# XuyangBai/PointDSC

Hardware: AMD Instinct MI355X
Metric: point-cloud pairs/sec @ N=5000 corr (higher is better)
Workload: dtype f32 (attention products as fp16x3 split (fp16 hi+lo operand pairs, three f16 MFMAs per product), f32 accumulate; fc_message / PointCN products as fp16 hi+lo split; spatial-consistency matrix stored as unorm16); 1 GPU; 3DMatch-like synthetic correspondences (BASELINE.json configs[2]): N=5000 corr, 32 pairs per step sharded over 1 GPU(s) = 32 per GPU, 12-layer PointDSC, seeded random weights; num_corr=5000, pairs_per_gpu=32, global_batch=32, compat_format=u16, layer_gemm=h3, att_leaves=canonical, latency_mode=False, range_guard=lazy (pipeline), collective=none (single process, no process group)

## Files before the change

### include/pointdsc_hip.h

```cpp
#ifndef POINTDSC_HIP_H
#define POINTDSC_HIP_H

#include <stddef.h>

#ifdef __cplusplus
extern "C" {
#endif

#define PDSC_VERSION 9
#define PDSC_CHANNELS 128
#define PDSC_MAX_K 64
#define PDSC_MAX_POWER_ITERS 32

enum pdsc_status {
    PDSC_OK = 0,
    PDSC_ERR_ARG = -1,
    PDSC_ERR_WORKSPACE = -2,
    PDSC_ERR_LAUNCH = -3
};

typedef struct pdsc_config {
    int in_dim;
    int num_layers;
    int num_channels;
// ... 84 lines not shown
    PDSC_LAYER_KERNEL_AUTO = 0,
    PDSC_LAYER_KERNEL_BLOCK,
    PDSC_LAYER_KERNEL_WAVE,
    PDSC_LAYER_KERNEL_H3,
    PDSC_LAYER_KERNEL_X3
};
typedef struct pdsc_layer_call {
    const float* msg;
    const float* part_o;
    const float* part_ml;
    int nsplit, Npad;
    const float* res;
    const float* feat_in;
    float* feat_out;
    float* featB_out;
    float* qkv_out;
    void* q_split;
    void* kv_tiles;
    const void* w1; const float* b1;
    const void* w2; const float* b2;
    const void* w3; const float* b3;
    const void* wp; const float* bp;
    const void* wq; const float* bq;
    const void* wq_split;
    const void* wfrag_tail;
    const void* wfrag_head;
    int gemm_format;
    int io_flags;
    int bs, N;
    int kernel;
} pdsc_layer_call;
int pdsc_layer_run(const pdsc_layer_call* call, void* stream);

size_t    pdsc_wsplit_bytes(const pdsc_config* cfg);
long long pdsc_wsplit_offset(const pdsc_config* cfg, int section, int layer);
int       pdsc_wsplit_build(const pdsc_config* cfg, const float* wpack, void* wsplit, void* stream);
#define PDSC_WS_FRAG_TAIL 100
#define PDSC_WS_FRAG_HEAD 101
#define PDSC_WS_FRAG_TAIL_H3 102
#define PDSC_WS_FRAG_HEAD_H3 103
#define PDSC_WS_FOLD_TAIL_H3 104
#define PDSC_WS_FOLD_HEAD_H3 105
#define PDSC_WS_FOLD_W 106
size_t pdsc_wfrag_fold_tail_bytes(void);
size_t pdsc_wfrag_fold_head_bytes(void);
int pdsc_layer_prefers_block(int bs, int N);
int pdsc_layer_h3_uses_coop(int bs, int N);
size_t pdsc_wfrag_tail_bytes(void);
size_t pdsc_wfrag_head_bytes(void);
int pdsc_wfrag_build_tail(const float* w1, const float* b1, const float* w2, const float* b2, const float* w3,
                          const float* b3, void* out, int gemm_format, void* stream);
int pdsc_wfrag_build_head(const float* wp, const float* bp, const float* wq, const float* bq, void* out,
                          int gemm_format, void* stream);

size_t pdsc_attention_scratch_bytes(int bs, int N, int nsplit);
int    pdsc_attention_default_split(int bs, int N);
int    pdsc_sc_attention(const float* qkv, const float* compat, long long ld, float* msg,
                         void* scratch, size_t scratch_bytes, int bs, int N, int nsplit, void* stream);

size_t pdsc_split_q_bytes(int bs, int N);
size_t pdsc_split_kv_bytes(int bs, int N);
int    pdsc_pack_qkv_split(const float* qkv, void* q_split, void* kv_tiles, int bs, int N, void* stream);
size_t pdsc_attention_split_scratch_bytes(int bs, int N, int nsplit);
int    pdsc_attention_split_default_split(int bs, int N);
int    pdsc_attention_leaf_count(int N);
int    pdsc_attention_leaf_plan(int bs, int N, int leaves_mode, int* nsplit, int* nleaf);
// ... 247 lines not shown
```

### pointdsc_amd/_lib.py

```python
from __future__ import annotations

import ctypes as C
import os
from pathlib import Path

PKG = Path(__file__).resolve().parent
LIB_PATH = Path(os.environ.get("POINTDSC_HIP_LIB", PKG / "libpointdsc_hip.so"))


class PointDSCLibraryError(RuntimeError):
    pass


class PdscConfig(C.Structure):
    _fields_ = [
        ("in_dim", C.c_int), ("num_layers", C.c_int), ("num_channels", C.c_int),
        ("num_iterations", C.c_int), ("k", C.c_int), ("refine_iters", C.c_int),
        ("inlier_threshold", C.c_float), ("nms_radius", C.c_float), ("refine_threshold", C.c_float),
        ("attention_precision", C.c_int), ("compat_format", C.c_int), ("layer_gemm", C.c_int),
        ("att_leaves", C.c_int), ("value_fold", C.c_int),
    ]


W_SECTIONS = [
    "LAYER0_W", "LAYER0_B", "PCN_W", "PCN_B", "QKV_W", "QKV_B", "FC1_W", "FC1_B", "FC2_W", "FC2_B",
    "FC3_W", "FC3_B", "CLS1_W", "CLS1_B", "CLS2_W", "CLS2_B", "CLS3_W", "CLS3_B", "SIGMA", "SIGMA_SPAT",
]
W = {name: i for i, name in enumerate(W_SECTIONS)}

_vp, _i, _f, _ll, _sz = C.c_void_p, C.c_int, C.c_float, C.c_longlong, C.c_size_t
_cfgp = C.POINTER(PdscConfig)


class PdscLayerCall(C.Structure):
    _fields_ = (
        [(n, _vp) for n in ("msg", "part_o", "part_ml")] + [("nsplit", _i), ("Npad", _i)] +
        [(n, _vp) for n in ("res", "feat_in", "feat_out", "featB_out", "qkv_out", "q_split", "kv_tiles",
                            "w1", "b1", "w2", "b2", "w3", "b3", "wp", "bp", "wq", "bq", "wq_split", "wfrag_tail", "wfrag_head")] +
        [(n, _i) for n in ("gemm_format", "io_flags", "bs", "N", "kernel")])

SIGNATURES = {
    "pdsc_version": (_i, []),
    "pdsc_set_range_report": (_i, [_vp]),
    "pdsc_last_error": (C.c_char_p, []),
    "pdsc_experiments_enabled": (_i, []),
    "pdsc_wpack_floats": (_ll, [_cfgp]),
    "pdsc_wpack_offset": (_ll, [_cfgp, _i, _i]),
    "pdsc_compat_ld": (_ll, [_i]),
    "pdsc_workspace_bytes": (_sz, [_cfgp, _i, _i, _i]),
    "pdsc_workspace_offset": (_ll, [_cfgp, _i, _i, _i, C.c_char_p]),
    "pdsc_spatial_compat": (_i, [_vp, _vp, _vp, _vp, _vp, _ll, _i, _i, _vp]),
    "pdsc_spatial_compat_u16": (_i, [_vp, _vp, _vp, _vp, _ll, _i, _i, _vp]),
    "pdsc_selftest_exact_math": (_i, [_vp, _f, _vp, _vp, _ll, _vp]),
    "pdsc_selftest_mfma_valu_neighbour": (_i, [_vp, _i, _i, _vp]),
    "pdsc_classifier_hidden": (_i, [_vp, _vp, _vp, _vp, _vp, _vp, _i, _vp]),
    "pdsc_linear": (_i, [_vp, _ll, _vp, _vp, _vp, _ll, _vp, _ll, _i, _i, _i, _i, _vp]),
    "pdsc_layer0": (_i, [_vp, _i, _vp, _vp, _vp, _i, _vp]),
    "pdsc_layer_run": (_i, [C.POINTER(PdscLayerCall), _vp]),
    "pdsc_wsplit_bytes": (_sz, [_cfgp]),
    "pdsc_wsplit_offset": (_ll, [_cfgp, _i, _i]),
    "pdsc_wsplit_build": (_i, [_cfgp, _vp, _vp, _vp]),
    "pdsc_layer_prefers_block": (_i, [_i, _i]),
    "pdsc_layer_h3_uses_coop": (_i, [_i, _i]),
    "pdsc_wfrag_tail_bytes": (_sz, []),
    "pdsc_wfrag_head_bytes": (_sz, []),
    "pdsc_wfrag_fold_tail_bytes": (_sz, []),
    "pdsc_wfrag_fold_head_bytes": (_sz, []),
    "pdsc_wfrag_build_tail": (_i, [_vp] * 7 + [_i, _vp]),
    "pdsc_wfrag_build_head": (_i, [_vp] * 5 + [_i, _vp]),
    "pdsc_sc_attention_split_partials": (_i, [_vp, _vp, _vp, _i, _ll, _vp, _sz, _i, _i, _i, _i, _vp]),
    "pdsc_split_q_bytes": (_sz, [_i, _i]),
    "pdsc_split_kv_bytes": (_sz, [_i, _i]),
    "pdsc_pack_qkv_split": (_i, [_vp, _vp, _vp, _i, _i, _vp]),
    "pdsc_attention_split_scratch_bytes": (_sz, [_i, _i, _i]),
    "pdsc_attention_split_default_split": (_i, [_i, _i]),
    "pdsc_attention_leaf_count": (_i, [_i]),
    "pdsc_attention_leaf_plan": (_i, [_i, _i, _i, C.POINTER(C.c_int), C.POINTER(C.c_int)]),
    "pdsc_attention_leaf_scratch_bytes": (_sz, [_i, _i, _i]),
    "pdsc_attention_trace": (_i, [_vp]),
    "pdsc_attention_leaf_split_override": (_i, [_i]),
    "pdsc_layer_trace": (_i, [_vp]),
    "pdsc_sc_attention_split": (_i, [_vp, _vp, _vp, _ll, _vp, _vp, _sz, _i, _i, _i, _vp]),
    "pdsc_sc_attention_split_u16": (_i, [_vp, _vp, _vp, _ll, _vp, _vp, _sz, _i, _i, _i, _vp]),
    "pdsc_attention_scratch_bytes": (_sz, [_i, _i, _i]),
    "pdsc_attention_default_split": (_i, [_i, _i]),
    "pdsc_sc_attention": (_i, [_vp, _vp, _ll, _vp, _vp, _sz, _i, _i, _i, _vp]),
    "pdsc_normalize_confidence": (_i, [_vp, _vp, _vp, _vp, _vp, _vp, _i, _vp]),
    "pdsc_nms_keys": (_i, [_vp, _vp, _f, _vp, _i, _i, _vp]),
    "pdsc_nms_workspace_bytes": (_sz, [_i, _i]),
    "pdsc_nms_keys_grid": (_i, [_vp, _vp, _f, _vp, _vp, _sz, _i, _i, _vp]),
    "pdsc_rank_select": (_i, [_vp, _vp, _i, _i, _i, _vp]),
# ... 115 lines not shown
```

### pointdsc_amd/csrc/layer.hip

```cpp
#include <stdlib.h>
#include <type_traits>
#include "pdsc_common.h"
#include "split_layout.h"
#include "merge_partials.h"
#include "layer_args.h"
#include "layer_block.h"

namespace pdsc {

constexpr int LF_ROWS = 32;
constexpr int LF_LD = PDSC_CHANNELS + 4;
constexpr int LF_TILE = LF_ROWS * LF_LD;


#define LF_STAMP(k)                                                                                   \
    if (a.trace && lane == 0) a.trace[(((size_t)blockIdx.y * gridDim.x + blockIdx.x) * 4 + wave) * 16 + (k)] = __builtin_readcyclecounter();

template <int K>
__device__ __forceinline__ void load_w(const float* __restrict__ W, int n0, int l31, int h, f32x4 (&w)[K / 8]) {
    const float* p = W + (size_t)(n0 + l31) * K + 4 * h;
#pragma unroll
    for (int q = 0; q < K / 8; ++q) w[q] = *reinterpret_cast<const f32x4*>(p + 8 * q);
}

// ... 321 lines not shown
        profile_mark_end(PDSC_PROF_LAYER, st);
        return rc;
    }
    if (tail) return launch_layer<true, false>(a, st);
    return launch_layer<false, true>(a, st);
}

}

static bool choose_layer_kernel(const pdsc_layer_call& c, const pdsc::LayerArgs& a, pdsc::LayerKernel* kernel) {
    using pdsc::LayerKernel;
    switch (c.kernel) {
        case PDSC_LAYER_KERNEL_BLOCK: *kernel = LayerKernel::Block; return true;
        case PDSC_LAYER_KERNEL_WAVE: *kernel = LayerKernel::Wave; return true;
        case PDSC_LAYER_KERNEL_H3: *kernel = LayerKernel::H3; return true;
        case PDSC_LAYER_KERNEL_X3: *kernel = LayerKernel::X3; return true;
        case PDSC_LAYER_KERNEL_AUTO: break;
        default: return false;
    }
    if (!a.wf_tail && !a.wf_head) {
        const char* ev = pdsc::env_str("PDSC_LAYER_VARIANT");
        const bool block = ev && (ev[0] == 'b' || ev[0] == 'w') ? ev[0] == 'b' : pdsc_layer_prefers_block(c.bs, c.N) != 0;
        *kernel = block ? LayerKernel::Block : LayerKernel::Wave;
    } else if (c.io_flags != 0) {
        *kernel = LayerKernel::H3;
    } else {
        const bool h3 = c.gemm_format == PDSC_LAYER_GEMM_H3 && pdsc::env_int("PDSC_LAYER_H3_VARIANT", 1) != 0 &&
                        pdsc::launch_layer_h3_fits(a, a.msg != nullptr || a.part_o != nullptr, a.featB_out != nullptr);
        *kernel = h3 ? LayerKernel::H3 : LayerKernel::Wave;
    }
    return true;
}

extern "C" int pdsc_layer_run(const pdsc_layer_call* call, void* stream) {
    PDSC_REQUIRE(call, "pdsc_layer_run: null call");
    const pdsc_layer_call& c = *call;
    const bool natural = c.w1 || c.b1 || c.w2 || c.b2 || c.w3 || c.b3 || c.wp || c.bp || c.wq || c.bq || c.wq_split;
    PDSC_REQUIRE(!natural || (!c.wfrag_tail && !c.wfrag_head), "pdsc_layer_run: weights given in natural layout AND as fragment streams");
    if (c.featB_out && !c.q_split && !c.kv_tiles) PDSC_REQUIRE(c.qkv_out, "pdsc_layer_run: head needs qkv_out when no split streams are given");
    pdsc::LayerArgs a = pdsc::layer_args_from_call(c);
    a.trace = c.io_flags ? nullptr : g_layer_trace;
    pdsc::LayerKernel kernel;
    PDSC_REQUIRE(choose_layer_kernel(c, a, &kernel), "pdsc_layer_run: kernel=%d", c.kernel);
    const int rc = pdsc::validate_layer_args(a, kernel, "pdsc_layer_run");
    return rc != PDSC_OK ? rc : pdsc::dispatch_layer(a, kernel, (hipStream_t)stream);
}
```

### pointdsc_amd/csrc/layer_h3.hip

```cpp
#include <stdlib.h>
#include <type_traits>
#include "pdsc_common.h"
#include "split_layout.h"
#include "merge_partials.h"
#include "layer_args.h"
#include "layer_wave.h"

namespace pdsc {

constexpr int PDSC_H3_COOP_TILES = 2560;

#define LH_STAMP(k) \
    if (TRACE && lane == 0) a.trace[(size_t)gw * 64 + (k)] = __builtin_readcyclecounter();

template <bool F = false>
constexpr int stage_tiles(int stage) { return stage == ST_FC1 || stage == ST_FC2 ? 2 : stage == ST_FC3 || stage == ST_PCN ? 4 : F ? 10 : 12; }

template <bool T, bool H, bool TRACE = false, int PIPE = 6, int EXP = 0, bool FB_PF = false, int NWV = LW_WAVES, int NBUF = 2, bool F = false>
__global__ __launch_bounds__(64 * NWV, NBUF > 2 ? 1 : 2) void layer_h3_kernel(LayerArgs a) {
    __shared__ __attribute__((aligned(16))) float Vs_all[NWV][32 * LW_VLD];
    const int lane = threadIdx.x & 63;
    const int wave = __builtin_amdgcn_readfirstlane(threadIdx.x >> 6);
    const int l31 = lane & 31, h = lane >> 5;
    const int tpp = ceil_div_dev(a.N, 32);
    const int gw = blockIdx.x * NWV + wave;
    if (gw >= a.bs * tpp) return;
    const int b = gw / tpp, tile = gw - b * tpp;
    const int m0 = b * a.N + tile * 32;
    const int valid = min(32, (a.nvalid ? a.nvalid[b] : a.N) - tile * 32);
    if (valid <= 0) return;
    const bool live = l31 < valid;
    const size_t row = (size_t)m0 + min(l31, valid - 1);
    float* Vs = Vs_all[wave];
    unsigned char* patch = reinterpret_cast<unsigned char*>(Vs);

    if (a.stagger_cycles > 0 && blockIdx.x < 512) {
        unsigned hwid;
        asm volatile("s_getreg_b32 %0, hwreg(HW_REG_HW_ID)" : "=s"(hwid));
        const bool late = a.stagger_mode == 1 ? (hwid & 1u) : a.stagger_mode == 2 ? (blockIdx.x & 1) : ((blockIdx.x >> 8) & 1);
        if (late) {
            const long long t0 = __builtin_readcyclecounter();
            while (__builtin_readcyclecounter() - t0 < a.stagger_cycles) __builtin_amdgcn_s_sleep(32);
        }
    }
    LH_STAMP(0)
    float rmax = 0.f;
    constexpr int NCH = num_chunks<T, H, F>();
    constexpr int VW = F ? LW_FOLD_VW : PDSC_CHANNELS;
    constexpr int NQ = VW / 8;
    WChunk w[NBUF];
    static_for<0, NBUF - 1>([&](auto jc) {
        constexpr int j = decltype(jc)::value;
        if constexpr (j < NCH) load_chunk<T, true, true, F>(w[j], a, j, lane);
    });

    u32x4 a0h[8], a0l[8], a1h[4], a1l[4], a2h[4], a2l[4], ayh[8], ayl[8], xqh[8], xql[8];
    f32x4 y3[16];
    if (T) {
        f32x4 x0[16];
        auto first_operand = [&](int kk) __attribute__((always_inline)) {
            if constexpr (F) {
                const float* bpr = reinterpret_cast<const float*>(a.wf_tail + LW_FOLD_BPRIME_BYTES);
#pragma unroll
                for (int u = 0; u < 2; ++u) {
                    const f32x4 bv = *reinterpret_cast<const f32x4*>(bpr + 8 * (2 * kk + u) + 4 * h);
#pragma unroll
                    for (int e = 0; e < 4; ++e) x0[2 * kk + u][e] = fmaxf(x0[2 * kk + u][e] + bv[e], 0.f);
                }
                make_kstep<true>(x0[2 * kk], x0[2 * kk + 1], a1h[kk], a1l[kk], rmax);
            } else {
                make_kstep<true>(x0[2 * kk], x0[2 * kk + 1], a0h[kk], a0l[kk], rmax);
            }
        };
        if (a.msg) {
#pragma unroll
            for (int q = 0; q < NQ; ++q) x0[q] = *reinterpret_cast<const f32x4*>(a.msg + row * VW + 8 * q + 4 * h);
#pragma unroll
            for (int kk = 0; kk < NQ / 2; ++kk) first_operand(kk);
        } else {
            with_split_count<MERGE_MAX_SPLIT_H3>(a.nsplit, [&](auto ns_tag) {
                constexpr int NS = decltype(ns_tag)::value;
                constexpr int GQ = (NS <= 2 ? 16 : NS <= 4 ? 8 : 4) < NQ ? (NS <= 2 ? 16 : NS <= 4 ? 8 : 4) : NQ;
                const size_t slot0 = (size_t)b * a.part_slots * a.Npad + (row - (size_t)b * a.N);
                const bool pf = a.io_flags & PDSC_IO_PARTIALS_PF;
                const size_t e0 = pf ? ((size_t)b * a.part_slots * a.Npad + (size_t)tile * 32) * VW + lane * 4 : slot0 * VW + 4 * h;
                const int eq = pf ? 256 : 8;
                const MergeWeights<NS> mw = merge_row_weights<NS>(a.part_ml, slot0, (size_t)a.Npad);
#pragma unroll
// ... 82 lines not shown
                        if constexpr (!(EXP & (2 | 16))) k_chunk_store(img, lane, 4 * (d.tile - 4) + s, ck);
                        else asm volatile("" :: "v"(ck));
                    }
                } else if constexpr (d.tile < 4) {
                    if constexpr (s < 4) {
                        unsigned hi[2], lo[2];
                        split4(v[s], hi, lo);
                        *reinterpret_cast<u32x4*>(patch + l31 * LW_PROW + 64 * h + 16 * s) = chunk_for_store(hi, lo);
                    }
                    if constexpr (s == 3) wave_lds_sync();
                    if constexpr (s >= 4) {
                        const int pt = 8 * (s - 4) + (lane >> 3), piece = lane & 7;
                        sp16* dst = a.qs + ((size_t)m0 + min(pt, valid - 1)) * SPL_Q_LD + (piece >> 2) * PDSC_CHANNELS + n0 + 8 * (piece & 3);
                        if constexpr (!(EXP & (2 | 8))) *reinterpret_cast<u32x4*>(dst) = ev;
                        else asm volatile("" :: "v"(ev), "v"(dst));
                    }
                    if constexpr (s >= 3 && s < 7) ev = patch_line(patch, lane, s - 3);
                } else {
                    if constexpr (s < 4) vt_put(Vs, lane, s, zero_unless(live, v[s]));
                    if constexpr (s == 3) wave_lds_sync();
                    if constexpr (s == 4 || s == 6) vt_gather(Vs, lane, (s - 4) >> 1, vt);
                    if constexpr (s == 5 || s == 7) {
                        u32x4 ch, cl;
                        vt_split(vt, ch, cl);
                        const int off = vt_offset<VW>(lane, (s - 5) >> 1, 32 * (d.tile - 8));
                        if constexpr (!(EXP & (2 | 32))) vt_store<VW>(img, off, ch, cl);
                        else asm volatile("" :: "v"(ch), "v"(cl), "v"(off));
                    }
                }
            }
        }
    };

    static_for<0, NCH>([&](auto ic) {
        constexpr int i = decltype(ic)::value;
        constexpr ChunkDesc d = chunk_desc<T, F>(i);
        if constexpr (i + NBUF - 1 < NCH && !((EXP & 1) && i >= 1)) load_chunk<T, true, true, F>(w[(i + NBUF - 1) % NBUF], a, i + NBUF - 1, lane);
        if constexpr (T && d.stage == ST_FC2 && d.tile == 0 && !(EXP & 4)) {
            const bool pf = a.io_flags & PDSC_IO_RES_PF;
            const float* r0 = a.res + (pf ? (size_t)gw * PF_TILE_FLOATS + lane * 4 : row * PDSC_CHANNELS + 4 * h);
            const int eq = pf ? 256 : 8;
#pragma unroll
            for (int q = 0; q < 16; ++q) y3[q] = *reinterpret_cast<const f32x4*>(r0 + eq * q);
        }
        const WChunk& wc = w[i % NBUF];
        if constexpr (d.chunk == 0) acc = bias_step(wc);
        constexpr bool pending = d.tile > 0;
        using StageC = std::integral_constant<int, d.stage>;
        using PrevC = std::integral_constant<int, d.tile - 1>;
        static_for<0, 4>([&](auto gc) {
            constexpr int g = decltype(gc)::value;
            if constexpr (d.stage == ST_QKV) {
                const sp16x8 wh = __builtin_bit_cast(sp16x8, wc.v[2 * g]), wl = __builtin_bit_cast(sp16x8, wc.v[2 * g + 1]);
                const sp16x8 bh = __builtin_bit_cast(sp16x8, xqh[4 * d.chunk + g]), bl = __builtin_bit_cast(sp16x8, xql[4 * d.chunk + g]);
                acc = PDSC_MFMA_X3(wl, bh, acc, 0, 0, 0);
                acc = PDSC_MFMA_X3(wh, bl, acc, 0, 0, 0);
                acc = PDSC_MFMA_X3(wh, bh, acc, 0, 0, 0);
            } else {
                const u32x4* oh = d.stage == ST_FC1 ? a0h : d.stage == ST_FC2 ? a1h : d.stage == ST_FC3 ? a2h : ayh;
                const u32x4* ol = d.stage == ST_FC1 ? a0l : d.stage == ST_FC2 ? a1l : d.stage == ST_FC3 ? a2l : ayl;
                const f32x16 zero = {0.f, 0.f, 0.f, 0.f, 0.f, 0.f, 0.f, 0.f, 0.f, 0.f, 0.f, 0.f, 0.f, 0.f, 0.f, 0.f};
                const f16x8 wh = __builtin_bit_cast(f16x8, wc.v[2 * g]), wl = __builtin_bit_cast(f16x8, wc.v[2 * g + 1]);
                const f16x8 bh = __builtin_bit_cast(f16x8, oh[4 * d.chunk + g]), bl = __builtin_bit_cast(f16x8, ol[4 * d.chunk + g]);
                cross = __builtin_amdgcn_mfma_f32_32x32x16_f16(wl, bh, (d.chunk == 0 && g == 0) ? zero : cross, 0, 0, 0);
                acc = __builtin_amdgcn_mfma_f32_32x32x16_f16(wh, bh, acc, 0, 0, 0);
                cross = __builtin_amdgcn_mfma_f32_32x32x16_f16(wh, bl, cross, 0, 0, 0);
            }
            if constexpr (pending) {
                if constexpr (d.nchunks == 2) {
                    epi(StageC{}, PrevC{}, std::integral_constant<int, 4 * d.chunk + g>{}, vp);
                } else {
                    epi(StageC{}, PrevC{}, std::integral_constant<int, 2 * g>{}, vp);
                    epi(StageC{}, PrevC{}, std::integral_constant<int, 2 * g + 1>{}, vp);
                }
            }
        });
        if constexpr (d.chunk == d.nchunks - 1) {
#pragma unroll
            for (int g = 0; g < 4; ++g)
#pragma unroll
                for (int e = 0; e < 4; ++e) vp[g][e] = d.stage != ST_QKV ? fmaf(cross[4 * g + e], H3_INV, acc[4 * g + e]) : acc[4 * g + e];
            if constexpr (d.tile == stage_tiles<F>(d.stage) - 1) {
                static_for<0, 8>([&](auto sc) { epi(StageC{}, std::integral_constant<int, d.tile>{}, sc, vp); });
            }
        }
        if constexpr (PIPE > 0) {
#pragma unroll
            for (int k = 0; k < 13; ++k) {
                __builtin_amdgcn_sched_group_barrier(0x008, 1, 0);
                __builtin_amdgcn_sched_group_barrier(0x002, PIPE, 0);
            }
        }
        LH_STAMP(2 + i)
        __builtin_amdgcn_sched_barrier(0);
    });

    LH_STAMP(63)
    range_report(a.range_flag, b, rmax);
}

bool launch_layer_h3_fits(const LayerArgs& a, bool tail, bool head) {
    if (a.gemm_format != PDSC_LAYER_GEMM_H3) return false;
    if (head && (!a.qs || !a.kv || a.qkv_out)) return false;
    if (tail && head && a.feat_out) return false;
    if (tail && !head && !a.feat_out) return false;
    return a.wf_tail || !tail;
}

H3Form layer_h3_form(const LayerArgs& a, bool tail, bool head) {
    const bool fb_pf = a.io_flags & PDSC_IO_FEATB_PF;
    if (a.value_fold) {
        if (tail && head && fb_pf) return H3Form::FoldTailHeadPF;
        if (head && !tail && fb_pf) return H3Form::FoldHeadPF;
        if (tail && !head) return H3Form::FoldTail;
        set_error("pdsc_layer_run(h3): the folded layer exists with point-fragment featB only");
        return H3Form::Unserved;
    }
    if (head && fb_pf) return tail ? H3Form::TailHeadPF : H3Form::HeadPF;
    return tail && head ? H3Form::TailHead : tail ? H3Form::Tail : H3Form::Head;
}

static void h3_launch_shape(int tiles, int* nwv, int* nbuf) {
    *nwv = LW_WAVES; *nbuf = 2;
    (void)tiles;
#ifdef PDSC_EXPERIMENTS
    const int force = env_int("PDSC_LAYER_H3_SHAPE", 0);
    if (force == 42 || force == 23 || force == 13 || force == 24 || force == 14 || force == 22) { *nwv = force / 10; *nbuf = force % 10; }
#endif
}

int launch_layer_h3(const LayerArgs& a, bool tail, bool head, hipStream_t st) {
    const int waves = a.bs * ceil_div(a.N, 32);
    int nwv, nbuf;
    h3_launch_shape(waves, &nwv, &nbuf);
    if (a.value_fold) { nwv = LW_WAVES; nbuf = 2; }
    const dim3 grid(ceil_div(waves, nwv)), block(64 * nwv);
    const H3Form form = layer_h3_form(a, tail, head);
    if (form == H3Form::Unserved) return PDSC_ERR_ARG;
    const bool timed = tail && head;
    int coop_tiles = PDSC_H3_COOP_TILES;
#ifdef PDSC_EXPERIMENTS
    coop_tiles = env_int("PDSC_LAYER_H3_COOP", coop_tiles);
#endif
    if (waves <= coop_tiles && !a.trace) {
        if (timed) profile_mark_begin(PDSC_PROF_LAYER, st);
        const int rc = launch_layer_h3_coop(a, tail, head, st);
        if (timed) profile_mark_end(PDSC_PROF_LAYER, st);
        return rc;
    }
    if (timed) profile_mark_begin(PDSC_PROF_LAYER, st);
#ifdef PDSC_EXPERIMENTS
#define PDSC_H3_LAUNCH_EXTRA(TT, HH, PF)                                                                                            \
        if (nwv == 1 && nbuf == 4) hipLaunchKernelGGL((layer_h3_kernel<TT, HH, false, 6, 0, PF, 1, 4>), grid, block, 0, st, a);      \
        else if (nwv == 2 && nbuf == 3) hipLaunchKernelGGL((layer_h3_kernel<TT, HH, false, 6, 0, PF, 2, 3>), grid, block, 0, st, a); \
        else if (nwv == 1 && nbuf == 3) hipLaunchKernelGGL((layer_h3_kernel<TT, HH, false, 6, 0, PF, 1, 3>), grid, block, 0, st, a); \
        else if (nwv == 2 && nbuf == 4) hipLaunchKernelGGL((layer_h3_kernel<TT, HH, false, 6, 0, PF, 2, 4>), grid, block, 0, st, a); \
        else if (nwv == 2 && nbuf == 2) hipLaunchKernelGGL((layer_h3_kernel<TT, HH, false, 6, 0, PF, 2, 2>), grid, block, 0, st, a); \
        else
#else
#define PDSC_H3_LAUNCH_EXTRA(TT, HH, PF)
#endif
#define PDSC_H3_LAUNCH(TT, HH, PF)                                                                                                  \
    do {                                                                                                                            \
        PDSC_H3_LAUNCH_EXTRA(TT, HH, PF)                                                                                            \
        hipLaunchKernelGGL((layer_h3_kernel<TT, HH, false, 6, 0, PF>), grid, block, 0, st, a);                                       \
    } while (0)
    switch (form) {
        case H3Form::FoldTailHeadPF: hipLaunchKernelGGL((layer_h3_kernel<true, true, false, 6, 0, true, LW_WAVES, 2, true>), grid, block, 0, st, a); break;
        case H3Form::FoldHeadPF: hipLaunchKernelGGL((layer_h3_kernel<false, true, false, 6, 0, true, LW_WAVES, 2, true>), grid, block, 0, st, a); break;
        case H3Form::FoldTail: hipLaunchKernelGGL((layer_h3_kernel<true, false, false, 6, 0, false, LW_WAVES, 2, true>), grid, block, 0, st, a); break;
        case H3Form::TailHeadPF: {
#ifdef PDSC_LAYER_DIAG
            const int ex = env_int("PDSC_LAYER_H3_EXP", 0);
            if (ex == 1) hipLaunchKernelGGL((layer_h3_kernel<true, true, false, 6, 1, true>), grid, block, 0, st, a);
            else if (ex == 2) hipLaunchKernelGGL((layer_h3_kernel<true, true, false, 6, 2, true>), grid, block, 0, st, a);
            else if (ex == 4) hipLaunchKernelGGL((layer_h3_kernel<true, true, false, 6, 4, true>), grid, block, 0, st, a);
            else if (ex == 7) hipLaunchKernelGGL((layer_h3_kernel<true, true, false, 6, 7, true>), grid, block, 0, st, a);
            else if (ex == 8) hipLaunchKernelGGL((layer_h3_kernel<true, true, false, 6, 8, true>), grid, block, 0, st, a);
            else if (ex == 16) hipLaunchKernelGGL((layer_h3_kernel<true, true, false, 6, 16, true>), grid, block, 0, st, a);
            else if (ex == 32) hipLaunchKernelGGL((layer_h3_kernel<true, true, false, 6, 32, true>), grid, block, 0, st, a);
            else if (ex == 64) hipLaunchKernelGGL((layer_h3_kernel<true, true, false, 6, 64, true>), grid, block, 0, st, a);
            else
#endif
            PDSC_H3_LAUNCH(true, true, true);
            break;
        }
        case H3Form::HeadPF: PDSC_H3_LAUNCH(false, true, true); break;
        case H3Form::TailHead:
#ifdef PDSC_EXPERIMENTS
            if (a.trace) hipLaunchKernelGGL((layer_h3_kernel<true, true, true>), dim3(ceil_div(waves, LW_WAVES)), dim3(64 * LW_WAVES), 0, st, a);
            else
#endif
            PDSC_H3_LAUNCH(true, true, false);
            break;
        case H3Form::Tail: PDSC_H3_LAUNCH(true, false, false); break;
        case H3Form::Head: PDSC_H3_LAUNCH(false, true, false); break;
        case H3Form::Unserved: break;
    }
#undef PDSC_H3_LAUNCH
#undef PDSC_H3_LAUNCH_EXTRA
    if (timed) profile_mark_end(PDSC_PROF_LAYER, st);
    return check_launch("pdsc_layer_run(h3)");
}

}

using namespace pdsc;

extern "C" int pdsc_layer_h3_uses_coop(int bs, int N) {
    if (bs <= 0 || N <= 0) return 0;
    int coop_tiles = PDSC_H3_COOP_TILES;
#ifdef PDSC_EXPERIMENTS
    coop_tiles = env_int("PDSC_LAYER_H3_COOP", coop_tiles);
#endif
    return (long long)bs * ceil_div(N, 32) <= coop_tiles ? 1 : 0;
}
```

### pointdsc_amd/csrc/layer_wave.h

```cpp
#pragma once
#include <type_traits>
#include "pdsc_common.h"
#include "split_layout.h"
#include "merge_partials.h"
#include "layer_args.h"

namespace pdsc {

constexpr int LW_WAVES = 4;
constexpr int LW_VLD = 36;
constexpr int LW_QKV_BUFS = 4;
#ifndef LW_H3_BUFS
#define LW_H3_BUFS 3
#endif

struct WChunk {
    f32x4 v[8];
    float bias;
};

template <int B, int E, class F>
__device__ __forceinline__ void static_for(F&& f) {
    if constexpr (B < E) {
        f(std::integral_constant<int, B>{});
// ... 57 lines not shown
    const int bias_tile = d.chunk == 0 ? tile_ordinal<F>(d) : -1;
    static_assert(FRAG || !F, "the folded layer takes fragment streams");
    if (FRAG) {
        if (T && i < tail_chunks<F>()) load_chunk_frag(w, a.wf_tail, i, tail_chunks<F>(), bias_tile, lane);
        else load_chunk_frag(w, a.wf_head, i - (T ? tail_chunks<F>() : 0), head_chunks<F>(), bias_tile, lane);
        return;
    }
    const int l31 = lane & 31, h = lane >> 5;
    const int n = 32 * d.tile + l31;
    if (d.chunk == 0) {
        const float* b = d.stage == ST_FC1 ? a.b1 : d.stage == ST_FC2 ? a.b2 : d.stage == ST_FC3 ? a.b3 : d.stage == ST_PCN ? a.bp : a.bq;
        const float bv = b[n];
        w.bias = h ? 0.f : bv;
    }
    switch (d.stage) {
        case ST_FC1: load_rows_f32(w, a.w1 + (size_t)n * 128 + 64 * d.chunk + 4 * h); break;
        case ST_FC2: load_rows_f32(w, a.w2 + (size_t)n * 64 + 4 * h); break;
        case ST_FC3: load_rows_f32(w, a.w3 + (size_t)n * 64 + 4 * h); break;
        case ST_PCN: load_rows_f32(w, a.wp + (size_t)n * 128 + 64 * d.chunk + 4 * h); break;
        default:
            if (X3) {
                const sp16* p = a.wq_split + (size_t)n * PDSC_CHANNELS + 64 * d.chunk + 8 * h;
#pragma unroll
                for (int k = 0; k < 4; ++k) {
                    w.v[2 * k] = *reinterpret_cast<const f32x4*>(p + 16 * k);
                    w.v[2 * k + 1] = *reinterpret_cast<const f32x4*>(p + (size_t)3 * PDSC_CHANNELS * PDSC_CHANNELS + 16 * k);
                }
            } else {
                load_rows_f32(w, a.wq + (size_t)n * 128 + 64 * d.chunk + 4 * h);
            }
    }
}

__device__ __forceinline__ void mma_f32(f32x16& acc, const WChunk& w, const f32x4* x) {
#pragma unroll
    for (int q = 0; q < 8; ++q)
#pragma unroll
        for (int e = 0; e < 4; ++e) acc = __builtin_amdgcn_mfma_f32_32x32x2f32(w.v[q][e], x[q][e], acc, 0, 0, 0);
}

__device__ __forceinline__ f32x16 bias_step(const WChunk& w) {
    const f32x16 zero = {0.f, 0.f, 0.f, 0.f, 0.f, 0.f, 0.f, 0.f, 0.f, 0.f, 0.f, 0.f, 0.f, 0.f, 0.f, 0.f};
    return __builtin_amdgcn_mfma_f32_32x32x2f32(w.bias, 1.0f, zero, 0, 0, 0);
}

__device__ __forceinline__ void mma_x3(f32x16& acc, const WChunk& w, const u32x4* xh, const u32x4* xl) {
#pragma unroll
    for (int i = 0; i < 4; ++i) {
        const sp16x8 wh = __builtin_bit_cast(sp16x8, w.v[2 * i]), wl = __builtin_bit_cast(sp16x8, w.v[2 * i + 1]);
        const sp16x8 bh = __builtin_bit_cast(sp16x8, xh[i]), bl = __builtin_bit_cast(sp16x8, xl[i]);
        acc = PDSC_MFMA_X3(wl, bh, acc, 0, 0, 0);
        acc = PDSC_MFMA_X3(wh, bl, acc, 0, 0, 0);
        acc = PDSC_MFMA_X3(wh, bh, acc, 0, 0, 0);
    }
}

__device__ __forceinline__ unsigned pack2(sp16 a, sp16 b) {
    return (unsigned)__builtin_bit_cast(unsigned short, a) | ((unsigned)__builtin_bit_cast(unsigned short, b) << 16);
}

typedef float f32x2 __attribute__((ext_vector_type(2)));

__device__ __forceinline__ void split2(float x0, float x1, unsigned& hi, unsigned& lo) { split_sp16_pair(x0, x1, hi, lo); }

__device__ __forceinline__ void split4(const f32x4& v, unsigned (&hi)[2], unsigned (&lo)[2]) {
    split2(v[0], v[1], hi[0], lo[0]);
    split2(v[2], v[3], hi[1], lo[1]);
}

typedef _Float16 f16x2 __attribute__((ext_vector_type(2)));
typedef _Float16 f16x8 __attribute__((ext_vector_type(8)));
constexpr float H3_SCALE = 2048.0f, H3_INV = 1.0f / 2048.0f;

__device__ __forceinline__ void split2h(float x0, float x1, unsigned& hi, unsigned& lo) {
    const f16x2 hv = __builtin_convertvector(f32x2{x0, x1}, f16x2);
    hi = __builtin_bit_cast(unsigned, hv);
    const f32x2 hf = __builtin_convertvector(hv, f32x2);
// ... 129 lines not shown
```

Baseline: 2555 pairs/s.

## Stream H3 layer weight chunks through an LDS ring via global_load_lds DMA

The H3 layer kernel no longer has each wave load every weight chunk into its own registers. The four waves of a block now cooperatively DMA each chunk into a four-slot LDS ring with global_load_lds, wait on vmcnt plus a barrier, and then read the hi/lo fragments from LDS one group ahead of use. Biases are also staged into LDS once per block. This cuts redundant per-wave global weight traffic and register pressure. In exchange it adds block-wide barriers, and idle waves must keep issuing their share of the DMA. The multi-shape experimental launch variants are removed, and a diagnostic entry point plus a coop-threshold override are added.

Result: no change. 2579 pairs/s (median of 6 runs) (+0.9%).

```diff
diff --git a/include/pointdsc_hip.h b/include/pointdsc_hip.h
--- a/include/pointdsc_hip.h
+++ b/include/pointdsc_hip.h
@@ -140,6 +140,14 @@
 } pdsc_layer_call;
 int pdsc_layer_run(const pdsc_layer_call* call, void* stream);
 
+typedef struct pdsc_layer_diag {
+    int value_fold, part_slots;
+    const int* nvalid;
+    unsigned int* range_flag;
+} pdsc_layer_diag;
+int pdsc_layer_run_diag(const pdsc_layer_call* call, const pdsc_layer_diag* diag, void* stream);
+int pdsc_layer_h3_coop_override(int tiles);
+
 size_t    pdsc_wsplit_bytes(const pdsc_config* cfg);
 long long pdsc_wsplit_offset(const pdsc_config* cfg, int section, int layer);
 int       pdsc_wsplit_build(const pdsc_config* cfg, const float* wpack, void* wsplit, void* stream);
diff --git a/pointdsc_amd/_lib.py b/pointdsc_amd/_lib.py
--- a/pointdsc_amd/_lib.py
+++ b/pointdsc_amd/_lib.py
@@ -38,6 +38,10 @@
         [(n, _vp) for n in ("res", "feat_in", "feat_out", "featB_out", "qkv_out", "q_split", "kv_tiles",
                             "w1", "b1", "w2", "b2", "w3", "b3", "wp", "bp", "wq", "bq", "wq_split", "wfrag_tail", "wfrag_head")] +
         [(n, _i) for n in ("gemm_format", "io_flags", "bs", "N", "kernel")])
+
+class PdscLayerDiag(C.Structure):
+    _fields_ = [("value_fold", _i), ("part_slots", _i), ("nvalid", _vp), ("range_flag", _vp)]
+
 
 SIGNATURES = {
     "pdsc_version": (_i, []),
@@ -57,6 +61,8 @@
     "pdsc_linear": (_i, [_vp, _ll, _vp, _vp, _vp, _ll, _vp, _ll, _i, _i, _i, _i, _vp]),
     "pdsc_layer0": (_i, [_vp, _i, _vp, _vp, _vp, _i, _vp]),
     "pdsc_layer_run": (_i, [C.POINTER(PdscLayerCall), _vp]),
+    "pdsc_layer_run_diag": (_i, [C.POINTER(PdscLayerCall), C.POINTER(PdscLayerDiag), _vp]),
+    "pdsc_layer_h3_coop_override": (_i, [_i]),
     "pdsc_wsplit_bytes": (_sz, [_cfgp]),
     "pdsc_wsplit_offset": (_ll, [_cfgp, _i, _i]),
     "pdsc_wsplit_build": (_i, [_cfgp, _vp, _vp, _vp]),
diff --git a/pointdsc_amd/csrc/layer.hip b/pointdsc_amd/csrc/layer.hip
--- a/pointdsc_amd/csrc/layer.hip
+++ b/pointdsc_amd/csrc/layer.hip
@@ -377,7 +377,16 @@
     return true;
 }
 
-extern "C" int pdsc_layer_run(const pdsc_layer_call* call, void* stream) {
+static int layer_run(const pdsc_layer_call* call, const pdsc_layer_diag* diag, void* stream);
+extern "C" int pdsc_layer_run(const pdsc_layer_call* call, void* stream) { return layer_run(call, nullptr, stream); }
+extern "C" int pdsc_layer_run_diag(const pdsc_layer_call* call, const pdsc_layer_diag* diag, void* stream) {
+    PDSC_REQUIRE(diag, "pdsc_layer_run_diag: null diag");
+    PDSC_REQUIRE((diag->value_fold == 0 || diag->value_fold == 1) && diag->part_slots >= 0, "pdsc_layer_run_diag: value_fold=%d part_slots=%d",
+                 diag->value_fold, diag->part_slots);
+    return layer_run(call, diag, stream);
+}
+
+static int layer_run(const pdsc_layer_call* call, const pdsc_layer_diag* diag, void* stream) {
     PDSC_REQUIRE(call, "pdsc_layer_run: null call");
     const pdsc_layer_call& c = *call;
     const bool natural = c.w1 || c.b1 || c.w2 || c.b2 || c.w3 || c.b3 || c.wp || c.bp || c.wq || c.bq || c.wq_split;
@@ -385,6 +394,12 @@
     if (c.featB_out && !c.q_split && !c.kv_tiles) PDSC_REQUIRE(c.qkv_out, "pdsc_layer_run: head needs qkv_out when no split streams are given");
     pdsc::LayerArgs a = pdsc::layer_args_from_call(c);
     a.trace = c.io_flags ? nullptr : g_layer_trace;
+    if (diag) {
+        a.value_fold = diag->value_fold;
+        if (diag->part_slots) a.part_slots = diag->part_slots;
+        a.nvalid = diag->nvalid;
+        a.range_flag = diag->range_flag;
+    }
     pdsc::LayerKernel kernel;
     PDSC_REQUIRE(choose_layer_kernel(c, a, &kernel), "pdsc_layer_run: kernel=%d", c.kernel);
     const int rc = pdsc::validate_layer_args(a, kernel, "pdsc_layer_run");
diff --git a/pointdsc_amd/csrc/layer_h3.hip b/pointdsc_amd/csrc/layer_h3.hip
--- a/pointdsc_amd/csrc/layer_h3.hip
+++ b/pointdsc_amd/csrc/layer_h3.hip
@@ -16,22 +16,65 @@
 template <bool F = false>
 constexpr int stage_tiles(int stage) { return stage == ST_FC1 || stage == ST_FC2 ? 2 : stage == ST_FC3 || stage == ST_PCN ? 4 : F ? 10 : 12; }
 
-template <bool T, bool H, bool TRACE = false, int PIPE = 6, int EXP = 0, bool FB_PF = false, int NWV = LW_WAVES, int NBUF = 2, bool F = false>
-__global__ __launch_bounds__(64 * NWV, NBUF > 2 ? 1 : 2) void layer_h3_kernel(LayerArgs a) {
-    __shared__ __attribute__((aligned(16))) float Vs_all[NWV][32 * LW_VLD];
+
+template <bool H, bool FB_PF>
+constexpr int epi_stores(int stage, int tile, int s) {
+    if (stage == ST_FC3) return !H && s < 4 ? 1 : 0;
+    if (stage == ST_PCN) return (FB_PF ? s < 4 : s >= 4) ? 1 : 0;
+    if (stage == ST_QKV) return tile < 4 ? (s >= 4 ? 1 : 0) : tile < 8 ? (s < 4 ? 1 : 0) : (s == 5 || s == 7 ? 2 : 0);
+    return 0;
+}
+template <bool T, bool H, bool F, bool FB_PF, int EXP>
+constexpr int chunk_vm_ops(int i) {
+    if (EXP != 0 || i < 0 || i >= num_chunks<T, H, F>()) return 0;
+    const ChunkDesc d = chunk_desc<T, F>(i);
+    int n = 0;
+    if (d.tile > 0)
+        for (int s = d.nchunks == 2 ? 4 * d.chunk : 0; s < (d.nchunks == 2 ? 4 * d.chunk + 4 : 8); ++s) n += epi_stores<H, FB_PF>(d.stage, d.tile - 1, s);
+    if (d.chunk == d.nchunks - 1 && d.tile == stage_tiles<F>(d.stage) - 1)
+        for (int s = 0; s < 8; ++s) n += epi_stores<H, FB_PF>(d.stage, d.tile, s);
+    return n;
+}
+template <bool T, bool H, bool F, int EXP>
+constexpr int chunk_pieces(int j) { return j >= 0 && j < num_chunks<T, H, F>() && (!(EXP & 1) || j < LH_RING - 1) ? LH_PIECES : 0; }
+template <bool T, bool H, bool F, bool FB_PF, int EXP>
+constexpr int ring_wait_count(int i, bool busy) {
+    if (i == 0) return 0;
+    return chunk_pieces<T, H, F, EXP>(i + 2) + (busy ? chunk_vm_ops<T, H, F, FB_PF, EXP>(i - 2) + chunk_vm_ops<T, H, F, FB_PF, EXP>(i - 1) : 0);
+}
+
+template <bool T, bool H, bool TRACE = false, int PIPE = 6, int EXP = 0, bool FB_PF = false, bool F = false>
+__global__ __launch_bounds__(64 * LW_WAVES, 2) void layer_h3_kernel(LayerArgs a) {
+    __shared__ __attribute__((aligned(16))) unsigned char smem[LH_LDS_BYTES];
     const int lane = threadIdx.x & 63;
     const int wave = __builtin_amdgcn_readfirstlane(threadIdx.x >> 6);
     const int l31 = lane & 31, h = lane >> 5;
+    constexpr int NCH = num_chunks<T, H, F>();
+    const unsigned lds_base = __builtin_amdgcn_readfirstlane((unsigned)(size_t)smem);
+    bias_issue<T, H, F>(a, lds_base, wave, lane);
+    static_for<0, LH_RING - 1>([&](auto jc) {
+        if constexpr (decltype(jc)::value < NCH) ring_issue<T, F>(a, decltype(jc)::value, lds_base, wave, lane);
+    });
     const int tpp = ceil_div_dev(a.N, 32);
-    const int gw = blockIdx.x * NWV + wave;
-    if (gw >= a.bs * tpp) return;
-    const int b = gw / tpp, tile = gw - b * tpp;
+    const int gw = blockIdx.x * LW_WAVES + wave;
+    int b = 0, tile = 0, valid = 0;
+    if (gw < a.bs * tpp) {
+        b = gw / tpp;
+        tile = gw - b * tpp;
+        valid = min(32, (a.nvalid ? a.nvalid[b] : a.N) - tile * 32);
+    }
+    if (valid <= 0) {
+        static_for<0, NCH>([&](auto ic) {
+            constexpr int i = decltype(ic)::value;
+            if constexpr (i + 1 < NCH) ring_wait_barrier<ring_wait_count<T, H, F, FB_PF, EXP>(i, false)>();
+            if constexpr (chunk_pieces<T, H, F, EXP>(i + LH_RING - 1) > 0) ring_issue<T, F>(a, i + LH_RING - 1, lds_base, wave, lane);
+        });
+        return;
+    }
     const int m0 = b * a.N + tile * 32;
-    const int valid = min(32, (a.nvalid ? a.nvalid[b] : a.N) - tile * 32);
-    if (valid <= 0) return;
     const bool live = l31 < valid;
     const size_t row = (size_t)m0 + min(l31, valid - 1);
-    float* Vs = Vs_all[wave];
+    float* Vs = reinterpret_cast<float*>(smem) + wave * (32 * LW_VLD);
     unsigned char* patch = reinterpret_cast<unsigned char*>(Vs);
 
     if (a.stagger_cycles > 0 && blockIdx.x < 512) {
@@ -45,15 +88,8 @@
     }
     LH_STAMP(0)
     float rmax = 0.f;
-    constexpr int NCH = num_chunks<T, H, F>();
     constexpr int VW = F ? LW_FOLD_VW : PDSC_CHANNELS;
     constexpr int NQ = VW / 8;
-    WChunk w[NBUF];
-    static_for<0, NBUF - 1>([&](auto jc) {
-        constexpr int j = decltype(jc)::value;
-        if constexpr (j < NCH) load_chunk<T, true, true, F>(w[j], a, j, lane);
-    });
-
     u32x4 a0h[8], a0l[8], a1h[4], a1l[4], a2h[4], a2l[4], ayh[8], ayl[8], xqh[8], xql[8];
     f32x4 y3[16];
     if (T) {
@@ -202,10 +238,17 @@
         }
     };
 
+    f32x4 wh_cur, wl_cur;
+    float bias_cur, bias_nxt = 0.f;
     static_for<0, NCH>([&](auto ic) {
         constexpr int i = decltype(ic)::value;
         constexpr ChunkDesc d = chunk_desc<T, F>(i);
-        if constexpr (i + NBUF - 1 < NCH && !((EXP & 1) && i >= 1)) load_chunk<T, true, true, F>(w[(i + NBUF - 1) % NBUF], a, i + NBUF - 1, lane);
+        if constexpr (i + 1 < NCH) ring_wait_barrier<ring_wait_count<T, H, F, FB_PF, EXP>(i, true)>();
+        if constexpr (chunk_pieces<T, H, F, EXP>(i + LH_RING - 1) > 0) ring_issue<T, F>(a, i + LH_RING - 1, lds_base, wave, lane);
+        if constexpr (i == 0) {
+            ring_read(smem, 0, 0, lane, wh_cur, wl_cur);
+            bias_cur = *reinterpret_cast<const float*>(smem + LH_BIAS_OFF + lane * 4);
+        }
         if constexpr (T && d.stage == ST_FC2 && d.tile == 0 && !(EXP & 4)) {
             const bool pf = a.io_flags & PDSC_IO_RES_PF;
             const float* r0 = a.res + (pf ? (size_t)gw * PF_TILE_FLOATS + lane * 4 : row * PDSC_CHANNELS + 4 * h);
@@ -213,15 +256,23 @@
 #pragma unroll
             for (int q = 0; q < 16; ++q) y3[q] = *reinterpret_cast<const f32x4*>(r0 + eq * q);
         }
-        const WChunk& wc = w[i % NBUF];
-        if constexpr (d.chunk == 0) acc = bias_step(wc);
+        if constexpr (d.chunk == 0) acc = bias_step(bias_cur);
         constexpr bool pending = d.tile > 0;
         using StageC = std::integral_constant<int, d.stage>;
         using PrevC = std::integral_constant<int, d.tile - 1>;
         static_for<0, 4>([&](auto gc) {
             constexpr int g = decltype(gc)::value;
+            f32x4 wh_nxt = wh_cur, wl_nxt = wl_cur;
+            if constexpr (g < 3) {
+                ring_read(smem, i % LH_RING, g + 1, lane, wh_nxt, wl_nxt);
+            } else if constexpr (i + 1 < NCH) {
+                ring_read(smem, (i + 1) % LH_RING, 0, lane, wh_nxt, wl_nxt);
+                constexpr ChunkDesc dn = chunk_desc<T, F>(i + 1);
+                constexpr int ord = tile_ordinal<F>(dn) + (T && i + 1 >= tail_chunks<F>() ? (F ? LW_FOLD_TAIL_TILES : LW_TAIL_TILES) : 0);
+                if constexpr (dn.chunk == 0) bias_nxt = *reinterpret_cast<const float*>(smem + LH_BIAS_OFF + ord * 256 + lane * 4);
+            }
             if constexpr (d.stage == ST_QKV) {
-                const sp16x8 wh = __builtin_bit_cast(sp16x8, wc.v[2 * g]), wl = __builtin_bit_cast(sp16x8, wc.v[2 * g + 1]);
+                const sp16x8 wh = __builtin_bit_cast(sp16x8, wh_cur), wl = __builtin_bit_cast(sp16x8, wl_cur);
                 const sp16x8 bh = __builtin_bit_cast(sp16x8, xqh[4 * d.chunk + g]), bl = __builtin_bit_cast(sp16x8, xql[4 * d.chunk + g]);
                 acc = PDSC_MFMA_X3(wl, bh, acc, 0, 0, 0);
                 acc = PDSC_MFMA_X3(wh, bl, acc, 0, 0, 0);
@@ -230,7 +281,7 @@
                 const u32x4* oh = d.stage == ST_FC1 ? a0h : d.stage == ST_FC2 ? a1h : d.stage == ST_FC3 ? a2h : ayh;
                 const u32x4* ol = d.stage == ST_FC1 ? a0l : d.stage == ST_FC2 ? a1l : d.stage == ST_FC3 ? a2l : ayl;
                 const f32x16 zero = {0.f, 0.f, 0.f, 0.f, 0.f, 0.f, 0.f, 0.f, 0.f, 0.f, 0.f, 0.f, 0.f, 0.f, 0.f, 0.f};
-                const f16x8 wh = __builtin_bit_cast(f16x8, wc.v[2 * g]), wl = __builtin_bit_cast(f16x8, wc.v[2 * g + 1]);
+                const f16x8 wh = __builtin_bit_cast(f16x8, wh_cur), wl = __builtin_bit_cast(f16x8, wl_cur);
                 const f16x8 bh = __builtin_bit_cast(f16x8, oh[4 * d.chunk + g]), bl = __builtin_bit_cast(f16x8, ol[4 * d.chunk + g]);
                 cross = __builtin_amdgcn_mfma_f32_32x32x16_f16(wl, bh, (d.chunk == 0 && g == 0) ? zero : cross, 0, 0, 0);
                 acc = __builtin_amdgcn_mfma_f32_32x32x16_f16(wh, bh, acc, 0, 0, 0);
@@ -244,7 +295,10 @@
                     epi(StageC{}, PrevC{}, std::integral_constant<int, 2 * g + 1>{}, vp);
                 }
             }
+            wh_cur = wh_nxt;
+            wl_cur = wl_nxt;
         });
+        bias_cur = bias_nxt;
         if constexpr (d.chunk == d.nchunks - 1) {
 #pragma unroll
             for (int g = 0; g < 4; ++g)
@@ -290,28 +344,19 @@
     return tail && head ? H3Form::TailHead : tail ? H3Form::Tail : H3Form::Head;
 }
 
-static void h3_launch_shape(int tiles, int* nwv, int* nbuf) {
-    *nwv = LW_WAVES; *nbuf = 2;
-    (void)tiles;
-#ifdef PDSC_EXPERIMENTS
-    const int force = env_int("PDSC_LAYER_H3_SHAPE", 0);
-    if (force == 42 || force == 23 || force == 13 || force == 24 || force == 14 || force == 22) { *nwv = force / 10; *nbuf = force % 10; }
-#endif
+static int g_h3_coop_override = -1;
+static int h3_coop_tiles() {
+    if (g_h3_coop_override >= 0) return g_h3_coop_override;
+    return env_int("PDSC_LAYER_H3_COOP", PDSC_H3_COOP_TILES);
 }
 
 int launch_layer_h3(const LayerArgs& a, bool tail, bool head, hipStream_t st) {
     const int waves = a.bs * ceil_div(a.N, 32);
-    int nwv, nbuf;
-    h3_launch_shape(waves, &nwv, &nbuf);
-    if (a.value_fold) { nwv = LW_WAVES; nbuf = 2; }
-    const dim3 grid(ceil_div(waves, nwv)), block(64 * nwv);
+    const dim3 grid(ceil_div(waves, LW_WAVES)), block(64 * LW_WAVES);
     const H3Form form = layer_h3_form(a, tail, head);
     if (form == H3Form::Unserved) return PDSC_ERR_ARG;
     const bool timed = tail && head;
-    int coop_tiles = PDSC_H3_COOP_TILES;
-#ifdef PDSC_EXPERIMENTS
-    coop_tiles = env_int("PDSC_LAYER_H3_COOP", coop_tiles);
-#endif
+    const int coop_tiles = h3_coop_tiles();
     if (waves <= coop_tiles && !a.trace) {
         if (timed) profile_mark_begin(PDSC_PROF_LAYER, st);
         const int rc = launch_layer_h3_coop(a, tail, head, st);
@@ -319,26 +364,18 @@
         return rc;
     }
     if (timed) profile_mark_begin(PDSC_PROF_LAYER, st);
-#ifdef PDSC_EXPERIMENTS
-#define PDSC_H3_LAUNCH_EXTRA(TT, HH, PF)                                                                                            \
-        if (nwv == 1 && nbuf == 4) hipLaunchKernelGGL((layer_h3_kernel<TT, HH, false, 6, 0, PF, 1, 4>), grid, block, 0, st, a);      \
-        else if (nwv == 2 && nbuf == 3) hipLaunchKernelGGL((layer_h3_kernel<TT, HH, false, 6, 0, PF, 2, 3>), grid, block, 0, st, a); \
-        else if (nwv == 1 && nbuf == 3) hipLaunchKernelGGL((layer_h3_kernel<TT, HH, false, 6, 0, PF, 1, 3>), grid, block, 0, st, a); \
-        else if (nwv == 2 && nbuf == 4) hipLaunchKernelGGL((layer_h3_kernel<TT, HH, false, 6, 0, PF, 2, 4>), grid, block, 0, st, a); \
-        else if (nwv == 2 && nbuf == 2) hipLaunchKernelGGL((layer_h3_kernel<TT, HH, false, 6, 0, PF, 2, 2>), grid, block, 0, st, a); \
-        else
-#else
-#define PDSC_H3_LAUNCH_EXTRA(TT, HH, PF)
+#define PDSC_H3_LAUNCH(TT, HH, PF) hipLaunchKernelGGL((layer_h3_kernel<TT, HH, false, 6, 0, PF>), grid, block, 0, st, a)
+    switch (form) {
+        case H3Form::FoldTailHeadPF:
+#ifdef PDSC_LAYER_DIAG
+            if (env_int("PDSC_LAYER_H3_EXP", 0) == 1) {
+                hipLaunchKernelGGL((layer_h3_kernel<true, true, false, 6, 1, true, true>), grid, block, 0, st, a);
+                break;
+            }
 #endif
-#define PDSC_H3_LAUNCH(TT, HH, PF)                                                                                                  \
-    do {                                                                                                                            \
-        PDSC_H3_LAUNCH_EXTRA(TT, HH, PF)                                                                                            \
-        hipLaunchKernelGGL((layer_h3_kernel<TT, HH, false, 6, 0, PF>), grid, block, 0, st, a);                                       \
-    } while (0)
-    switch (form) {
-        case H3Form::FoldTailHeadPF: hipLaunchKernelGGL((layer_h3_kernel<true, true, false, 6, 0, true, LW_WAVES, 2, true>), grid, block, 0, st, a); break;
-        case H3Form::FoldHeadPF: hipLaunchKernelGGL((layer_h3_kernel<false, true, false, 6, 0, true, LW_WAVES, 2, true>), grid, block, 0, st, a); break;
-        case H3Form::FoldTail: hipLaunchKernelGGL((layer_h3_kernel<true, false, false, 6, 0, false, LW_WAVES, 2, true>), grid, block, 0, st, a); break;
+            hipLaunchKernelGGL((layer_h3_kernel<true, true, false, 6, 0, true, true>), grid, block, 0, st, a); break;
+        case H3Form::FoldHeadPF: hipLaunchKernelGGL((layer_h3_kernel<false, true, false, 6, 0, true, true>), grid, block, 0, st, a); break;
+        case H3Form::FoldTail: hipLaunchKernelGGL((layer_h3_kernel<true, false, false, 6, 0, false, true>), grid, block, 0, st, a); break;
         case H3Form::TailHeadPF: {
 #ifdef PDSC_LAYER_DIAG
             const int ex = env_int("PDSC_LAYER_H3_EXP", 0);
@@ -358,7 +395,7 @@
         case H3Form::HeadPF: PDSC_H3_LAUNCH(false, true, true); break;
         case H3Form::TailHead:
 #ifdef PDSC_EXPERIMENTS
-            if (a.trace) hipLaunchKernelGGL((layer_h3_kernel<true, true, true>), dim3(ceil_div(waves, LW_WAVES)), dim3(64 * LW_WAVES), 0, st, a);
+            if (a.trace) hipLaunchKernelGGL((layer_h3_kernel<true, true, true>), grid, block, 0, st, a);
             else
 #endif
             PDSC_H3_LAUNCH(true, true, false);
@@ -368,7 +405,6 @@
         case H3Form::Unserved: break;
     }
 #undef PDSC_H3_LAUNCH
-#undef PDSC_H3_LAUNCH_EXTRA
     if (timed) profile_mark_end(PDSC_PROF_LAYER, st);
     return check_launch("pdsc_layer_run(h3)");
 }
@@ -379,9 +415,11 @@
 
 extern "C" int pdsc_layer_h3_uses_coop(int bs, int N) {
     if (bs <= 0 || N <= 0) return 0;
-    int coop_tiles = PDSC_H3_COOP_TILES;
-#ifdef PDSC_EXPERIMENTS
-    coop_tiles = env_int("PDSC_LAYER_H3_COOP", coop_tiles);
-#endif
-    return (long long)bs * ceil_div(N, 32) <= coop_tiles ? 1 : 0;
-}
+    return (long long)bs * ceil_div(N, 32) <= h3_coop_tiles() ? 1 : 0;
+}
+
+extern "C" int pdsc_layer_h3_coop_override(int tiles) {
+    PDSC_REQUIRE(tiles >= -1, "pdsc_layer_h3_coop_override: tiles=%d (-1 = the library's threshold, 0 = never, else a tile count)", tiles);
+    g_h3_coop_override = tiles;
+    return PDSC_OK;
+}
diff --git a/pointdsc_amd/csrc/layer_wave.h b/pointdsc_amd/csrc/layer_wave.h
--- a/pointdsc_amd/csrc/layer_wave.h
+++ b/pointdsc_amd/csrc/layer_wave.h
@@ -113,6 +113,60 @@
     }
 }
 
+constexpr int LH_RING = 4;
+constexpr int LH_PATCH_BYTES = LW_WAVES * 32 * LW_VLD * 4;
+constexpr int LH_RING_OFF = LH_PATCH_BYTES;
+constexpr int LH_BIAS_OFF = LH_RING_OFF + LH_RING * LW_CHUNK_BYTES;
+constexpr int LH_LDS_BYTES = LH_BIAS_OFF + (LW_TAIL_TILES + LW_HEAD_TILES) * 256;
+constexpr int LH_PIECES = LW_CHUNK_BYTES / 1024 / LW_WAVES;
+static_assert(LH_PIECES * LW_WAVES * 1024 == LW_CHUNK_BYTES && LH_LDS_BYTES <= 65536, "ring shape");
+
+__device__ __forceinline__ void lds_dma16(const unsigned char* base, unsigned voff, unsigned lds_dst) {
+    unsigned keep;
+    asm volatile("s_mov_b32 %0, m0\n\ts_mov_b32 m0, %3\n\ts_nop 0\n\tglobal_load_lds_dwordx4 %1, %2\n\ts_mov_b32 m0, %0"
+                 : "=&s"(keep) : "v"(voff), "s"(base), "s"(lds_dst) : "memory");
+}
+__device__ __forceinline__ void lds_dma4(const unsigned char* base, unsigned voff, unsigned lds_dst) {
+    unsigned keep;
+    asm volatile("s_mov_b32 %0, m0\n\ts_mov_b32 m0, %3\n\ts_nop 0\n\tglobal_load_lds_dword %1, %2\n\ts_mov_b32 m0, %0"
+                 : "=&s"(keep) : "v"(voff), "s"(base), "s"(lds_dst) : "memory");
+}
+
+template <bool T, bool F>
+__device__ __forceinline__ const unsigned char* chunk_source(const LayerArgs& a, int j) {
+    return T && j < tail_chunks<F>() ? a.wf_tail + (size_t)j * LW_CHUNK_BYTES : a.wf_head + (size_t)(j - (T ? tail_chunks<F>() : 0)) * LW_CHUNK_BYTES;
+}
+template <bool T, bool F>
+__device__ __forceinline__ void ring_issue(const LayerArgs& a, int j, unsigned lds_base, int wave, int lane) {
+    const unsigned char* src = chunk_source<T, F>(a, j) + wave * (LH_PIECES * 1024);
+    const unsigned dst = lds_base + LH_RING_OFF + (j % LH_RING) * LW_CHUNK_BYTES + wave * (LH_PIECES * 1024);
+#pragma unroll
+    for (int u = 0; u < LH_PIECES; ++u) lds_dma16(src + u * 1024, lane * 16, dst + u * 1024);
+}
+template <bool T, bool H, bool F>
+__device__ __forceinline__ void bias_issue(const LayerArgs& a, unsigned lds_base, int wave, int lane) {
+    constexpr int TT = T ? (F ? LW_FOLD_TAIL_TILES : LW_TAIL_TILES) : 0, HT = H ? (F ? LW_FOLD_HEAD_TILES : LW_HEAD_TILES) : 0;
+#pragma unroll
+    for (int u = 0; u < (TT + HT + LW_WAVES - 1) / LW_WAVES; ++u) {
+        const int t = wave + LW_WAVES * u;
+        if (t < TT + HT) {
+            const unsigned char* src = t < TT ? a.wf_tail + (size_t)tail_chunks<F>() * LW_CHUNK_BYTES + t * 256
+                                              : a.wf_head + (size_t)head_chunks<F>() * LW_CHUNK_BYTES + (t - TT) * 256;
+            lds_dma4(src, lane * 4, lds_base + LH_BIAS_OFF + t * 256);
+        }
+    }
+}
+template <int N>
+__device__ __forceinline__ void ring_wait_barrier() {
+    static_assert(N >= 0 && N < 64, "vmcnt is a 6-bit field");
+    asm volatile("s_waitcnt vmcnt(%0)\n\ts_barrier" ::"n"(N) : "memory");
+}
+__device__ __forceinline__ void ring_read(const unsigned char* smem, int slot, int g, int lane, f32x4& hi, f32x4& lo) {
+    const unsigned char* p = smem + LH_RING_OFF + slot * LW_CHUNK_BYTES + 2048 * g + lane * 16;
+    hi = *reinterpret_cast<const f32x4*>(p);
+    lo = *reinterpret_cast<const f32x4*>(p + 1024);
+}
+
 __device__ __forceinline__ void mma_f32(f32x16& acc, const WChunk& w, const f32x4* x) {
 #pragma unroll
     for (int q = 0; q < 8; ++q)
@@ -120,10 +174,11 @@
         for (int e = 0; e < 4; ++e) acc = __builtin_amdgcn_mfma_f32_32x32x2f32(w.v[q][e], x[q][e], acc, 0, 0, 0);
 }
 
-__device__ __forceinline__ f32x16 bias_step(const WChunk& w) {
+__device__ __forceinline__ f32x16 bias_step(float bias) {
     const f32x16 zero = {0.f, 0.f, 0.f, 0.f, 0.f, 0.f, 0.f, 0.f, 0.f, 0.f, 0.f, 0.f, 0.f, 0.f, 0.f, 0.f};
-    return __builtin_amdgcn_mfma_f32_32x32x2f32(w.bias, 1.0f, zero, 0, 0, 0);
-}
+    return __builtin_amdgcn_mfma_f32_32x32x2f32(bias, 1.0f, zero, 0, 0, 0);
+}
+__device__ __forceinline__ f32x16 bias_step(const WChunk& w) { return bias_step(w.bias); }
 
 __device__ __forceinline__ void mma_x3(f32x16& acc, const WChunk& w, const u32x4* xh, const u32x4* xl) {
 #pragma unroll
```
